# quokka-astro/quokka

Measured on AMD Instinct MI355X. Metric: Mcell-updates/s on 3D Sedov unigrid, higher is better.
Workload: dtype f64; 1 GPU; 3D Sedov blast 256x256x256 unigrid (tests/blast_unigrid_256.in scaled to 256^3 cells per GPU), 128^3 boxes, PPM+HLLC RK2, gamma=1.4, CFL 0.3, reflecting octant; cells_per_gpu=16777216, boxes_per_gpu=8, parallelism=box-decomposition x1, rk2_mode=carry, fofc_stages=0, retries=0, x_sweep_in_y_march=True

## Files before the change

quokka_amd/csrc/qk_hydro_fused.hip:

```cpp
#include "qk_device.hpp"
#include <algorithm>
#include <cmath>
#include <cstdlib>
#include <type_traits>
#include <vector>

#include "qk_internal.hpp"

using namespace qk;

namespace
{

constexpr int NG = 4;

template <class P> QK_DEV void streamStore(P *p, double v) { __builtin_nontemporal_store(v, p); }
template <class P> QK_DEV auto streamLoad(P *p) -> double { return __builtin_nontemporal_load(p); }

struct SGeom {
	int64_t off;
	int glo[3];
	int n[3];
	int pitch;
	int64_t ncell;
};

enum { S_AUX = 0, S_RHS = 4 };
constexpr auto scratchComps(int nscalars) -> int { return S_RHS + NVAR + nscalars + 1; }
constexpr int QK_FUSED_MAX_SCALARS = 3;

struct SweepArgs {
	const qk_box *boxes;
	const SGeom *geom;
	double *scratch;
	int64_t total_cells;
	const qk_array4 *U_in;
	const qk_array4 *U_old;
	qk_array4 *U_out;
	qk_array4 *halfFlux;
	qk_array4 *halfVel;
	qk_iarray4 *redoFlag;
	unsigned long long *redo_count;
	int *error_flag;
	double *max_signal;
	double inv_dx;
	double dx;
	double inv_dx0, dx0;
	double dx3[3];
	double dt;
	double densityFloor, tempFloor;
	double K_visc;
	int use_dual_energy;
	bool reconstruct_eint;
	bool same_old;
	bool store_rk2;
	qk_array4 *rk2Flux;
	qk_array4 *rhs1;
	const qk_carray4 *fluxMask;
	int nseg;
	bool prim_in, prim_out;
	bool store_vel;
	qk_array4 *rk2Vel;
};

QK_DEV auto sarr(SweepArgs const &a, int comp) -> double * { return a.scratch + static_cast<int64_t>(comp) * a.total_cells; }

#ifndef QK_PT_Y
#define QK_PT_Y 7
#define QK_PT_THREADS 512
#endif
constexpr int PT_X = 66, PT_Y = QK_PT_Y, PT_THREADS = QK_PT_THREADS;
constexpr int PT_OWN = PT_X * PT_Y;
constexpr int PT_HALO_Y = 6 * PT_X;
constexpr int PT_HALO = PT_HALO_Y + 6 * PT_Y;
static_assert(PT_HALO <= PT_THREADS && PT_OWN <= PT_THREADS, "one halo cell per thread");

struct PlaneCell {
	double rho, vx, vy, vz, P;
};

struct PlaneRaw {
	double rho, mx, my, mz, E;
};
QK_DEV auto planeLoad(RA4 const &U, int64_t u) -> PlaneRaw
{
	PlaneRaw r;
	r.rho = U.p[u + U.ns * RHO];
	r.mx = U.p[u + U.ns * MX];
	r.my = U.p[u + U.ns * MY];
	r.mz = U.p[u + U.ns * MZ];
	r.E = U.p[u + U.ns * ENE];
	return r;
}
QK_DEV auto planeCell(Eos const &eos, bool re, PlaneRaw const &r) -> PlaneCell
{
	PlaneCell c;
	c.rho = r.rho;
	const Recip R = recipOf(c.rho);
	c.vx = divBy(r.mx, R);
	c.vy = divBy(r.my, R);
	c.vz = divBy(r.mz, R);
	if (eos.isothermal) {
		c.P = c.rho * (eos.cs_iso * eos.cs_iso);
		return c;
	}
	const double kinetic_energy = 0.5 * c.rho * (c.vx * c.vx + c.vy * c.vy + c.vz * c.vz);
	const double Eint_cons = r.E - kinetic_energy;
	if (re) {
		const double e = divBy(Eint_cons, R);
		const double e2 = (c.rho == 0.0) ? 0.0 : divBy(c.rho * e, R);
		c.P = eos.gm1 * c.rho * e2;
	} else {
		const double e = (c.rho == 0.0) ? 0.0 : divBy(Eint_cons, R);
		c.P = eos.gm1 * c.rho * e;
	}
	return c;
}

QK_DEV auto chiCompressive(double Pm2, double Pm1, double Pp1, double Pp2, Recip const &RKS, Recip const &Rbeta) -> double
{
	constexpr double beta_max = 0.85;
	constexpr double Zmax = 0.75;
	constexpr double Zmin = 0.25;
	const double dP1 = fabs(Pp1 - Pm1);
	const double beta_denom = fabs(Pp2 - Pm2);
	const double beta = (beta_denom != 0) ? divBy(dP1, recipOf(beta_denom)) : 0;
	const double chi_min = smax0(smin1(divBy(beta_max - beta, Rbeta)));
	const double Z = divBy(dP1, RKS);
	return smax(chi_min, smin1((Zmax - Z) / (Zmax - Zmin)));
}

template <bool PRIM>
__global__ void __launch_bounds__(PT_THREADS, 4) k_pre3(const qk_box *boxes, const SGeom *geom, const qk_array4 *U_t, double *scratch, int64_t T, Eos eos, bool re, int nseg,
							    int xt, int yt, int ndim)
{
	constexpr bool prim_in = PRIM;
	const unsigned nblk = gridDim.x, lin = blockIdx.x;
	const unsigned q8 = nblk / 8, r8 = nblk % 8, xcd = lin % 8, slot = lin / 8;
	const unsigned logical = (xcd < r8) ? xcd * (q8 + 1) + slot : r8 * (q8 + 1) + (xcd - r8) * q8 + slot;
	const int bix = static_cast<int>(logical % xt), biy = static_cast<int>((logical / xt) % yt), biz = static_cast<int>(logical / (xt * yt));
	__shared__ double s_P[PT_Y + 6][PT_X + 6];
	__shared__ double s_vx[PT_Y][PT_X + 4], s_vy[PT_Y + 4][PT_X];
	__shared__ double s_cx[PT_Y][PT_X + 2], s_cy[PT_Y + 2][PT_X];

	const int b = biz / nseg;
	const int seg = biz - b * nseg;
	const qk_box bx = boxes[b];
	const SGeom g = geom[b];
	RA4 U(U_t[b]);
	const int t = threadIdx.x;
	const int x0 = bx.lo[0] - 1 + bix * PT_X;
	const int y0 = bx.lo[1] - 1 + biy * PT_Y;
	if (x0 > bx.hi[0] + 1 || y0 > bx.hi[1] + 1) {
		return;
	}
	const int nall = bx.hi[2] - bx.lo[2] + 3;
	const int seglen = (nall + nseg - 1) / nseg;
	const int zfirst = bx.lo[2] - 1 + seg * seglen;
	const int zlast = min(zfirst + seglen - 1, bx.hi[2] + 1);
	if (zlast < zfirst) {
		return;
	}
	const int ngy = (ndim >= 2) ? NG : 0, ngz = (ndim == 3) ? NG : 0;
	const int flo[2] = {bx.lo[0] - NG, bx.lo[1] - ngy}, fhi[2] = {bx.hi[0] + NG, bx.hi[1] + ngy};
	const int fzlo = bx.lo[2] - ngz, fzhi = bx.hi[2] + ngz;

	const bool own = t < PT_OWN;
	const int ty = own ? t / PT_X : 0;
	const int tx = own ? t - ty * PT_X : 0;
	const int oi = x0 + tx, oj = y0 + ty;
	const bool ownIn = own && oi <= fhi[0] && oj >= flo[1] && oj <= fhi[1];
	const bool ownOut = own && oi <= bx.hi[0] + 1 && oj <= bx.hi[1] + 1;
	const int h = t - (PT_THREADS - PT_HALO);
	int hx = 0, hy = 0;
	if (h >= 0) {
		if (h < PT_HALO_Y) {
			const int r = h / PT_X;
			hx = h - r * PT_X;
			hy = (r < 3) ? r - 3 : PT_Y + r - 3;
		} else {
			const int r = (h - PT_HALO_Y) / 6, c = (h - PT_HALO_Y) - r * 6;
			hy = r;
			hx = (c < 3) ? c - 3 : PT_X + c - 3;
		}
	}
	const int hi_ = x0 + hx, hj = y0 + hy;
	const bool haloIn = (h >= 0) && hi_ >= flo[0] && hi_ <= fhi[0] && hj >= flo[1] && hj <= fhi[1];
	const bool rimX = (h >= 0) && (hx == -1 || hx == PT_X);
	const bool rimY = (h >= 0) && (hy == -1 || hy == PT_Y);
	const int rx = hx, ry = hy;

	double Pz[5] = {1., 1., 1., 1., 1.}, vzw[5] = {0., 0., 0., 0., 0.}, rhoz[3] = {1., 1., 1.}, chz[3] = {1., 1., 1.};
	const Recip Rbeta = recipOf(0.85 - 0.75);
	double fm[4] = {1., 1., 1., 1.}, fdx[4] = {0., 0., 0., 0.}, fdy[4] = {0., 0., 0., 0.};
	double *Sout = scratch + g.off;
	const PlaneRaw neutral{1., 0., 0., 0., prim_in ? 1. : 1. / eos.gm1};
	auto cellOf = [&](PlaneRaw const &r) -> PlaneCell { return prim_in ? PlaneCell{r.rho, r.mx, r.my, r.mz, r.E} : planeCell(eos, re, r); };
	int64_t uo = ownIn ? U.idx(oi, oj, zfirst - 3) : 0;
	int64_t uh = haloIn ? U.idx(hi_, hj, zfirst - 3) : 0;

	for (int k = zfirst - 3; k <= zlast + 3; ++k, uo += U.ks, uh += U.ks) {
		const bool inPlane = (k >= zfirst) && (k <= zlast);
		const bool kIn = (k >= fzlo) && (k <= fzhi);
		const PlaneCell c = cellOf((ownIn && kIn) ? planeLoad(U, uo) : neutral);
#pragma unroll
		for (int m = 0; m < 4; ++m) {
			Pz[m] = Pz[m + 1];
			vzw[m] = vzw[m + 1];
		}
		Pz[4] = c.P;
		vzw[4] = c.vz;
		rhoz[0] = rhoz[1];
		rhoz[1] = rhoz[2];
		rhoz[2] = c.rho;
#pragma unroll
		for (int m = 0; m < 3; ++m) {
			fm[m] = fm[m + 1];
			fdx[m] = fdx[m + 1];
			fdy[m] = fdy[m + 1];
		}
		if (inPlane) {
			PlaneCell hc{1., 0., 0., 0., 1.};
			if (own) {
				s_P[ty + 3][tx + 3] = c.P;
				s_vx[ty][tx + 2] = c.vx;
				s_vy[ty + 2][tx] = c.vy;
			}
			if (h >= 0) {
				if constexpr (PRIM) {
					if (haloIn && kIn) {
						hc.P = U.p[uh + U.ns * ENE];
						if (hy >= 0 && hy < PT_Y && hx >= -2 && hx < PT_X + 2) {
							hc.vx = U.p[uh + U.ns * MX];
						}
						if (hx >= 0 && hx < PT_X && hy >= -2 && hy < PT_Y + 2) {
							hc.vy = U.p[uh + U.ns * MY];
						}
						if (rimX || rimY) {
							hc.rho = U.p[uh + U.ns * RHO];
						}
					}
				} else {
					hc = cellOf((haloIn && kIn) ? planeLoad(U, uh) : neutral);
				}
				s_P[hy + 3][hx + 3] = hc.P;
				if (hy >= 0 && hy < PT_Y && hx >= -2 && hx < PT_X + 2) {
					s_vx[hy][hx + 2] = hc.vx;
				}
				if (hx >= 0 && hx < PT_X && hy >= -2 && hy < PT_Y + 2) {
					s_vy[hy + 2][hx] = hc.vy;
				}
			}
			__syncthreads();
			if (own) {
				const bool cx = s_vx[ty][tx + 3] < s_vx[ty][tx + 1];
				const bool cy = (ndim >= 2) && (s_vy[ty + 3][tx] < s_vy[ty + 1][tx]);
				double chx = 1.0, chy = 1.0;
				if (cx || cy) {
					const Recip RKS = recipOf(flatteningKS(eos, c.rho, c.P));
					if (cx) {
						const double *Pr = &s_P[ty + 3][tx + 3];
						chx = chiCompressive(Pr[-2], Pr[-1], Pr[1], Pr[2], RKS, Rbeta);
					}
					if (cy) {
						chy = chiCompressive(s_P[ty + 1][tx + 3], s_P[ty + 2][tx + 3], s_P[ty + 4][tx + 3], s_P[ty + 5][tx + 3], RKS, Rbeta);
					}
				}
				s_cx[ty][tx + 1] = chx;
				s_cy[ty + 1][tx] = chy;
			}
			if (rimX) {
				double chx = 1.0;
				if (s_vx[ry][rx + 3] < s_vx[ry][rx + 1]) {
					const double *Pr = &s_P[ry + 3][rx + 3];
					chx = chiCompressive(Pr[-2], Pr[-1], Pr[1], Pr[2], recipOf(flatteningKS(eos, hc.rho, hc.P)), Rbeta);
				}
				s_cx[ry][rx + 1] = chx;
			} else if (rimY) {
				double chy = 1.0;
				if ((ndim >= 2) && (s_vy[ry + 3][rx] < s_vy[ry + 1][rx])) {
					chy = chiCompressive(s_P[ry + 1][rx + 3], s_P[ry + 2][rx + 3], s_P[ry + 4][rx + 3], s_P[ry + 5][rx + 3],
							     recipOf(flatteningKS(eos, hc.rho, hc.P)), Rbeta);
				}
				s_cy[ry + 1][rx] = chy;
			}
			__syncthreads();
			if (own) {
				const double mx = smin(smin(s_cx[ty][tx], s_cx[ty][tx + 1]), s_cx[ty][tx + 2]);
				const double my = smin(smin(s_cy[ty][tx], s_cy[ty + 1][tx]), s_cy[ty + 2][tx]);
				fm[3] = smin(mx, my);
				fdx[3] = smin(s_vx[ty][tx + 3] - c.vx, c.vx - s_vx[ty][tx + 1]);
				fdy[3] = smin(s_vy[ty + 3][tx] - c.vy, c.vy - s_vy[ty + 1][tx]);
			}
			__syncthreads();
		}
		chz[0] = chz[1];
		chz[1] = chz[2];
		chz[2] = 1.0;
		if ((ndim == 3) && (vzw[3] < vzw[1])) {
			chz[2] = chiCompressive(Pz[0], Pz[1], Pz[3], Pz[4], recipOf(flatteningKS(eos, rhoz[0], Pz[2])), Rbeta);
		}
		const int ko = k - 3;
		if (ko >= zfirst && ko <= zlast && ownOut) {
			const int64_t cc = (oi - g.glo[0]) + static_cast<int64_t>(g.pitch) * ((oj - g.glo[1]) + static_cast<int64_t>(g.n[1]) * (ko - g.glo[2]));
			Sout[(S_AUX + 0) * T + cc] = smin(fm[0], smin(smin(chz[0], chz[1]), chz[2]));
			Sout[(S_AUX + 1) * T + cc] = fdx[0];
			Sout[(S_AUX + 2) * T + cc] = fdy[0];
			Sout[(S_AUX + 3) * T + cc] = smin(vzw[2] - vzw[1], vzw[1] - vzw[0]);
		}
	}
}

template <int ORDER> QK_DEV void cellEdges(const double qm2, const double qm1, const double q0, const double qp1, const double qp2, double &am, double &ap)
{
	if (ORDER == 3) {
		ppmEdges(qm2, qm1, q0, qp1, qp2, am, ap);
	} else if (ORDER == 2) {
		plmEdges<QK_LIMITER_MINMOD>(qm1, q0, qp1, am, ap);
	} else {
		am = q0;
		ap = q0;
	}
}

QK_DEV void flattenEdges(double chi, double mean, double &am, double &ap)
{
	am = chi * am + (1. - chi) * mean;
	ap = chi * ap + (1. - chi) * mean;
}

template <int ORDER> QK_DEV void reconstructVar(double chi, double qm2, double qm1, double q0, double qp1, double qp2, double &am, double &ap)
{
	cellEdges<ORDER>(qm2, qm1, q0, qp1, qp2, am, ap);
	flattenEdges(chi, q0, am, ap);
}
template <int ORDER, int NV, class NB> QK_DEV void reconstructCell(double chi, const double (&q0)[NV], NB nb, double (&am)[NV], double (&ap)[NV])
{
#pragma unroll
	for (int n = 0; n < NV; ++n) {
		reconstructVar<ORDER>(chi, nb(-2, n), nb(-1, n), q0[n], nb(1, n), nb(2, n), am[n], ap[n]);
	}
}

template <int NV, int W> QK_DEV void getColumn(const double (*s)[W], int t, double (&v)[NV])
{
#pragma unroll
	for (int n = 0; n < NV; ++n) {
		v[n] = s[n][t];
	}
}
template <int NV, int W> QK_DEV void putColumn(double (*s)[W], int t, const double (&v)[NV])
{
#pragma unroll
	for (int n = 0; n < NV; ++n) {
		s[n][t] = v[n];
	}
}

template <int NS> QK_DEV void primsOf(RA4 const &U, int64_t u, Eos const &eos, bool re, bool prim_in, const double (&Uc)[NVAR], double (&q)[NVAR + NS])
{
	if (prim_in) {
#pragma unroll
		for (int n = 0; n < NVAR; ++n) {
			q[n] = Uc[n];
		}
	} else {
		consToPrim(eos, re, Uc, q);
	}
#pragma unroll
	for (int n = NVAR; n < NVAR + NS; ++n) {
		q[n] = U.p[u + U.ns * n];
	}
}
template <int NS> QK_DEV void loadPrims(RA4 const &U, int64_t u, Eos const &eos, bool re, bool prim_in, double (&q)[NVAR + NS], double (&Uc)[NVAR])
{
#pragma unroll
	for (int n = 0; n < NVAR; ++n) {
		Uc[n] = U.p[u + U.ns * n];
	}
	primsOf<NS>(U, u, eos, re, prim_in, Uc, q);
}

template <int DIR, int RIEMANN, bool TWOD, int NS>
QK_DEV void faceFluxAll(Eos const &eos, bool re, int ndim, const double (&qL)[NVAR + NS], const double (&qR)[NVAR + NS], double du, double dvl, double dvr, double dwl,
			double dwr, double K_visc, double (&F)[NVAR + NS], double &vf)
{
	Wave wv;
	faceFlux<DIR, RIEMANN, TWOD>(eos, re, ndim, qL, qR, du, dvl, dvr, dwl, dwr, K_visc, F, vf, NS > 0 ? &wv : nullptr);
#pragma unroll
	for (int n = NVAR; n < NVAR + NS; ++n) {
		F[n] = scalarFlux<RIEMANN>(wv, qL[n], qR[n]);
	}
}

using CA4 = A4<const char, qk_carray4>;
QK_DEV auto maskByte(qk_carray4 const &d, int i, int j, int k) -> int
{
	if (i < d.begin[0] || i >= d.end[0] || j < d.begin[1] || j >= d.end[1] || k < d.begin[2] || k >= d.end[2]) {
		return 0;
	}
	return CA4(d)(i, j, k);
}
template <int STAGE, int NV> QK_DEV void maskedFaceFlux(SweepArgs const &a, int b, int i, int j, int k, const double F[NV])
{
	if (STAGE == 1) {
		WA4 HF(a.halfFlux[b]);
		const int64_t o = HF.idx(i, j, k);
#pragma unroll
		for (int n = 0; n < NV; ++n) {
			HF.p[o + HF.ns * n] = F[n];
		}
	} else {
		RA4 HF(a.halfFlux[b]);
		WA4 RF(a.rk2Flux[b]);
		const int64_t o = HF.idx(i, j, k), o2 = RF.idx(i, j, k);
#pragma unroll
		for (int n = 0; n < NV; ++n) {
			RF.p[o2 + RF.ns * n] = 0.5 * HF.p[o + HF.ns * n] + 0.5 * F[n];
		}
	}
}

template <int NV> QK_DEV void loadF1(SweepArgs const &a, int b, const int (&fi)[3], double (&F1)[NV + 1])
{
	RA4 HF(a.halfFlux[b]);
	RA4 HV(a.halfVel[b]);
	const int64_t o = HF.idx(fi[0], fi[1], fi[2]);
#pragma unroll
	for (int n = 0; n < NV; ++n) {
		F1[n] = HF.p[o + HF.ns * n];
	}
	F1[NV] = HV(fi[0], fi[1], fi[2]);
}
template <int STAGE, bool CARRY, bool FOFC, int DIR, int NS, bool TWOD>
QK_DEV void settleFace(SweepArgs const &a, Eos const &eos, int ndim, int b, const int (&fi)[3], bool live, bool marked, const double (&F1)[NVAR + NS + 1],
		       const double (&qLo)[NVAR + NS], const double (&qRo)[NVAR + NS], double (&F)[NVAR + NS], double &vf)
{
	constexpr int NV = NVAR + NS;
	if (CARRY) {
		if (marked) {
			maskedFaceFlux<STAGE, NV>(a, b, fi[0], fi[1], fi[2], F);
		}
		return;
	}
	int fm[3] = {fi[0], fi[1], fi[2]};
	fm[DIR] -= 1;
	bool firstOrder = false;
	if constexpr (FOFC) {
		CIA4 flag(a.redoFlag[b]);
		firstOrder = (flag(fm[0], fm[1], fm[2]) != 0) || (flag(fi[0], fi[1], fi[2]) != 0);
	}
	if (STAGE == 2) {
#pragma unroll
		for (int n = 0; n < NV; ++n) {
			F[n] = 0.5 * F1[n] + 0.5 * F[n];
		}
		vf = 0.5 * F1[NV] + 0.5 * vf;
	}
	if constexpr (FOFC) {
		if (firstOrder) {
			if (STAGE == 1) {
				faceFluxAll<DIR, QK_RIEMANN_LLF, TWOD, NS>(eos, a.reconstruct_eint, ndim, qLo, qRo, 0., 0., 0., 0., 0., 0., F, vf);
			} else {
				RA4 Uold(a.U_old[b]);
				double qL[NV], qR[NV], Uc[NVAR];
				loadPrims<NS>(Uold, Uold.idx(fm[0], fm[1], fm[2]), eos, a.reconstruct_eint, false, qL, Uc);
				loadPrims<NS>(Uold, Uold.idx(fi[0], fi[1], fi[2]), eos, a.reconstruct_eint, false, qR, Uc);
				faceFluxAll<DIR, QK_RIEMANN_LLF, TWOD, NS>(eos, a.reconstruct_eint, ndim, qL, qR, 0., 0., 0., 0., 0., 0., F, vf);
			}
		}
	} else if (STAGE == 1) {
		if (live) {
			WA4 HF(a.halfFlux[b]);
			WA4 HV(a.halfVel[b]);
			const int64_t o = HF.idx(fi[0], fi[1], fi[2]);
#pragma unroll
			for (int n = 0; n < NV; ++n) {
				HF.p[o + HF.ns * n] = F[n];
			}
			HV(fi[0], fi[1], fi[2]) = vf;
		}
	}
	if (STAGE == 2 && a.store_rk2 && live) {
		WA4 RF(a.rk2Flux[b]);
		const int64_t o2 = RF.idx(fi[0], fi[1], fi[2]);
#pragma unroll
		for (int n = 0; n < NV; ++n) {
			RF.p[o2 + RF.ns * n] = F[n];
		}
	}
	if (STAGE == 2 && a.store_vel && live) {
		WA4 RV(a.rk2Vel[b]);
		RV(fi[0], fi[1], fi[2]) = vf;
	}
}

QK_DEV void reduceSignal(double *max_signal, double sig0, double sig1)
{
	for (int off = 32; off > 0; off >>= 1) {
		sig0 = smax(sig0, __shfl_xor(sig0, off));
		sig1 = smax(sig1, __shfl_xor(sig1, off));
	}
	if ((threadIdx.x & 63) == 0) {
		atomicMaxNonNeg(&max_signal[0], sig0);
		atomicMaxNonNeg(&max_signal[1], sig1);
	}
}
template <int NDIM> QK_DEV auto cellCentredDivV(RA4 const &U, int i, int j, int k, const double dx[3]) -> double
{
	auto vel = [&](int ii, int jj, int kk, int d) { return U(ii, jj, kk, MX + d) / U(ii, jj, kk, RHO); };
	double s = (vel(i + 1, j, k, 0) - vel(i - 1, j, k, 0)) / dx[0];
	if (NDIM >= 2) {
		s = s + (vel(i, j + 1, k, 1) - vel(i, j - 1, k, 1)) / dx[1];
	}
	if (NDIM == 3) {
		s = s + (vel(i, j, k + 1, 2) - vel(i, j, k - 1, 2)) / dx[2];
	}
	return 0.5 * s;
}

struct EpiConst {
	Recip RkB, RkBu, Rmu;
};
QK_DEV auto epiConst(Eos const &eos) -> EpiConst
{
	EpiConst c;
	c.RkB = eos.RkB;
	c.RkBu = eos.RkBu;
	c.Rmu = eos.Rmu;
	return c;
}
QK_DEV auto epiTgas(Eos const &eos, EpiConst const &ec, Recip const &Rrho, double Eint) -> double
{
	if (eos.tmodel == 1) {
		return sqrt(sqrt(4.0 * Eint / eos.alpha));
	}
	const double e = divBy(Eint, Rrho);
	const double T = divBy(e * eos.mu * Eos::m_u * eos.gm1, ec.RkB);
	return divBy(T * Eos::k_B, ec.RkBu);
}
QK_DEV auto epiEint(Eos const &eos, EpiConst const &ec, double rho, double T) -> double
{
	if (eos.tmodel == 1) {
		return (eos.alpha / 4.0) * ((T * T) * (T * T));
	}
	const double p = divBy(rho * T * Eos::k_B, ec.Rmu);
	const double e = p / (eos.gm1 * rho);
	return divBy(e * rho * eos.kB_user, ec.RkB);
}

template <int NS, int CS, bool FOFC = false, int NDIM = 3>
QK_DEV void updateCellFrom(SweepArgs const &a, Eos const &eos, EpiConst const &ec, int b, int i, int j, int k, double U[NVAR + NS], const double rhs_sweeps[NVAR + NS],
			   double div_v, const double half[NVAR + NS + 1], double &sig0, double &sig1, bool haveP = false, double Pknown = 0.)
{
	WA4 Un(a.U_out[b]);
	IA4 flag(a.redoFlag[b]);
	if constexpr (FOFC) {
		if (flag(i, j, k) != 0) {
			div_v = cellCentredDivV<NDIM>(RA4(a.U_old[b]), i, j, k, a.dx3);
		}
	}
	double rhs[NVAR + NS];
#pragma unroll
	for (int n = 0; n < NVAR + NS; ++n) {
		rhs[n] = rhs_sweeps[n];
	}
	double Pgas;
	if (CS == 2) {
		Pgas = half[NVAR + NS];
	} else if (haveP) {
		Pgas = Pknown;
	} else {
		const double rho = U[RHO];
		if (eos.isothermal) {
			Pgas = rho * eos.cs_iso * eos.cs_iso;
		} else {
			const Recip Ro = recipOf(rho);
			const double vx = divBy(U[MX], Ro), vy = divBy(U[MY], Ro), vz = divBy(U[MZ], Ro);
			const double thermal_energy = U[ENE] - 0.5 * rho * (vx * vx + vy * vy + vz * vz);
			const double e = (rho == 0.0) ? 0.0 : divBy(thermal_energy, Ro);
			Pgas = eos.gm1 * rho * e;
		}
	}
	double r[NVAR];
#pragma unroll
	for (int n = 0; n < NVAR; ++n) {
		r[n] = rhs[n];
	}
	r[EINT] += -Pgas * div_v;
	if (CS == 1) {
		WA4 R1(a.rhs1[b]);
		const int64_t c1 = R1.idx(i, j, k);
		const double hdt = 0.5 * a.dt;
#pragma unroll
		for (int n = 0; n < NVAR + NS; ++n) {
			streamStore(&R1.p[c1 + R1.ns * n], U[n] + hdt * ((n < NVAR) ? r[n] : rhs[n]));
		}
		streamStore(&R1.p[c1 + R1.ns * (NVAR + NS)], Pgas);
	}
	if (CS == 2) {
		const double hdt = 0.5 * a.dt;
#pragma unroll
		for (int n = 0; n < NVAR + NS; ++n) {
			U[n] = half[n] + hdt * ((n < NVAR) ? r[n] : rhs[n]);
		}
	} else {
#pragma unroll
		for (int n = 0; n < NVAR; ++n) {
			U[n] = U[n] + a.dt * r[n];
		}
#pragma unroll
		for (int n = NVAR; n < NVAR + NS; ++n) {
// ... 319 lines not shown
	pos[0] = i;
	pos[OT] = ot;
	pos[DIR] = lo - 3;
	int64_t c = (pos[0] - g.glo[0]) * st[0] + (pos[1] - g.glo[1]) * st[1] + (pos[2] - g.glo[2]) * st[2];
	const double *S = a.scratch + g.off;
	double *Sw = a.scratch + g.off;
	RA4 Uin(a.U_in[b]);
	RA4 Uold(a.U_old[b]);
	const EpiConst ec = epiConst(eos);
	int64_t u = Uin.idx(pos[0], pos[1], pos[2]);
	const int64_t ums = (DIR == 1) ? Uin.js : Uin.ks;

	constexpr int AV = Axes<DIR, TWOD>::v, AW = Axes<DIR, TWOD>::w;
	double q[5][NV];
	double apPrev[NV], Fprev[NV];
	double vfPrev = 0., dVprev = 0., dWprev = 0.;
	bool maskCol = false;
	int maskLo = 0, maskHi = -1;
	if (CARRY && a.fluxMask != nullptr) {
		const qk_carray4 md = a.fluxMask[b];
		maskCol = live && i >= md.begin[0] && i < md.end[0] && ot >= md.begin[OT] && ot < md.end[OT];
		maskLo = md.begin[DIR];
		maskHi = md.end[DIR] - 1;
	}
	constexpr bool RING = LAST && (STAGE == 1);
	__shared__ double s_ring[RING ? 3 : 1][RING ? NV : 1][RING ? 64 * MARCH_BY : 1];
	__shared__ double s_fx[FUSEX ? MARCH_BY : 1][FUSEX ? NV + 2 : 1][FUSEX ? XW : 1];
	__shared__ double s_edge[FUSEX ? MARCH_BY : 1][FUSEX ? XROWS : 1][6][FUSEX ? NV + 1 : 1];
	double chiPrev = 1.;
	const int lself = (FUSEX && threadIdx.x == 0) ? 69 : static_cast<int>(threadIdx.x) + 2;
	const int lnext = (FUSEX && threadIdx.x == 63) ? 68 : static_cast<int>(threadIdx.x) + 3;
	const int tid = threadIdx.y * 64 + threadIdx.x;
	const bool ring = RING && a.same_old;
	int slot = 0;
	double Uo[NV];
#pragma unroll
	for (int n = 0; n < NV; ++n) {
		apPrev[n] = 0.;
		Fprev[n] = 0.;
#pragma unroll
		for (int m = 0; m < 5; ++m) {
			q[m][n] = 0.;
		}
	}

	constexpr bool PFQ = !FUSEX && NS == 0;
	double Un[NVAR];
	if constexpr (PFQ) {
#pragma unroll
		for (int n = 0; n < NVAR; ++n) {
			Un[n] = Uin.p[u + Uin.ns * n];
		}
	}
	for (int step = 0; step < nvalid + 6; ++step, c += ms, u += ums) {
#pragma unroll
		for (int n = 0; n < NV; ++n) {
			q[0][n] = q[1][n];
			q[1][n] = q[2][n];
			q[2][n] = q[3][n];
			q[3][n] = q[4][n];
		}
		{
			double Uc[NVAR];
			if constexpr (PFQ) {
#pragma unroll
				for (int n = 0; n < NVAR; ++n) {
					Uc[n] = Un[n];
					Un[n] = Uin.p[u + ums + Uin.ns * n];
				}
				primsOf<NS>(Uin, u, eos, a.reconstruct_eint, a.prim_in, Uc, q[4]);
			} else {
				loadPrims<NS>(Uin, u, eos, a.reconstruct_eint, a.prim_in, q[4], Uc);
			}
			if constexpr (RING) {
				if (ring) {
#pragma unroll
					for (int n = 0; n < NV; ++n) {
						Uo[n] = s_ring[slot][n][tid];
						s_ring[slot][n][tid] = (n < NVAR) ? Uc[n] : q[4][n];
					}
					slot = (slot == 2) ? 0 : slot + 1;
				}
			}
		}
		if (step < 4) {
			continue;
		}
		const int64_t cc = c - 2 * ms;
		const double chi = S[(S_AUX + 0) * T + cc];
		const double dV = S[(S_AUX + 1 + AV) * T + cc];
		const double dW = S[(S_AUX + 1 + AW) * T + cc];
		int fidx[3], cidx[3];
		fidx[0] = cidx[0] = i;
		fidx[OT] = cidx[OT] = ot;
		fidx[DIR] = lo + (step - 5);
		cidx[DIR] = lo + (step - 6);
		const int64_t cu = cc - ms;
		double rhs_in[NV + 1], F1[NV + 1];
		if (step >= 6) {
			if constexpr (FUSEX) {
				double(*sx)[XW] = s_fx[threadIdx.y];
				EdgeRow<NV> *edge = s_edge[threadIdx.y];
				const int rr = (step - 6) & (XROWS - 1);
				if (rr == 0) {
					fusexEdgeBatch<ORDER, NS>(a, eos, Uin, g, st, S, bx.lo[0] + bix * 64, cidx[DIR], hi, ot, edge);
					waveFence();
					stageEdgeRow<NV>(sx, edge[0]);
				}
				const double Dy = S[(S_AUX + 2) * T + cu];
				const int l = static_cast<int>(threadIdx.x) + 2;
				putColumn(sx, l, q[1]);
				waveFence();
				double amx[NV], apx[NV];
				reconstructCell<ORDER>(chiPrev, q[1], [&](int m, int n) { return sx[n][l + m]; }, amx, apx);
				const double uLeft = sx[PVX][l - 1];
				waveFence();
				putColumn(sx, l, apx);
				sx[NV][l] = Dy;
				sx[NV + 1][l] = dVprev;
				waveFence();
				double qLx[NV], Fx[NV], vfx;
				getColumn(sx, l - 1, qLx);
				const double dvl = sx[NV][l - 1], dwl = sx[NV + 1][l - 1];
				faceFluxAll<0, QK_RIEMANN_HLLC, false, NS>(eos, a.reconstruct_eint, 3, qLx, amx, q[1][PVX] - uLeft, dvl, Dy, dwl, dVprev, a.K_visc, Fx, vfx);
				waveFence();
				putColumn(sx, l, Fx);
				sx[NV][l] = vfx;
				waveFence();
#pragma unroll
				for (int n = 0; n < NV; ++n) {
					rhs_in[n] = a.inv_dx0 * (sx[n][lself] - sx[n][lnext]);
				}
				rhs_in[NV] = (sx[NV][lnext] - sx[NV][lself]) / a.dx0;
				waveFence();
				if (rr + 1 < XROWS) {
					stageEdgeRow<NV>(sx, edge[rr + 1]);
				}
			} else {
#pragma unroll
				for (int n = 0; n < NV + 1; ++n) {
					rhs_in[n] = streamLoad(&S[(S_RHS + n) * T + cu]);
				}
			}
			if (LAST && !ring && !(CARRY && STAGE == 2)) {
				const int64_t co = Uold.idx(cidx[0], cidx[1], cidx[2]);
#pragma unroll
				for (int n = 0; n < NV; ++n) {
					Uo[n] = Uold.p[co + Uold.ns * n];
				}
			}
			if (CARRY && LAST && STAGE == 2) {
				RA4 R1(a.rhs1[b]);
				const int64_t c1 = R1.idx(cidx[0], cidx[1], cidx[2]);
#pragma unroll
				for (int n = 0; n < NV + 1; ++n) {
					F1[n] = R1.p[c1 + R1.ns * n];
				}
			}
		}
		if (!CARRY && STAGE == 2 && step >= 5) {
			loadF1<NV>(a, b, fidx, F1);
		}
		double am[NV], ap[NV];
		reconstructCell<ORDER>(chi, q[2], [&](int m, int n) { return q[2 + m][n]; }, am, ap);
		if (step >= 5) {
			const double du = q[2][PVX + DIR] - q[1][PVX + DIR];
			double F[NV], vf;
			faceFluxAll<DIR, QK_RIEMANN_HLLC, TWOD, NS>(eos, a.reconstruct_eint, TWOD ? 2 : 3, apPrev, am, du, dVprev, dV, dWprev, dW, a.K_visc, F, vf);
			bool marked = false;
			if (maskCol && fidx[DIR] >= maskLo && cidx[DIR] <= maskHi) {
				CA4 M(a.fluxMask[b]);
				const int m0 = (cidx[DIR] >= maskLo) ? M(cidx[0], cidx[1], cidx[2]) : 0;
				const int m1 = (fidx[DIR] <= maskHi) ? M(fidx[0], fidx[1], fidx[2]) : 0;
				marked = (m0 | m1) != 0;
			}
			settleFace<STAGE, CARRY, FOFC, DIR, NS, TWOD>(a, eos, TWOD ? 2 : 3, b, fidx, live, marked, F1, q[1], q[2], F, vf);
			if (step >= 6) {
				double rhs[NV];
#pragma unroll
				for (int n = 0; n < NV; ++n) {
					rhs[n] = rhs_in[n] + a.inv_dx * (Fprev[n] - F[n]);
				}
				const double div_v = rhs_in[NV] + (vf - vfPrev) / a.dx;
				if (LAST) {
					if (live) {
						updateCellFrom<NS, CARRY ? STAGE : 0, FOFC, TWOD ? 2 : 3>(a, eos, ec, b, cidx[0], cidx[1], cidx[2], Uo, rhs, div_v, F1, sig0, sig1,
													    (STAGE == 1) && a.same_old && !a.reconstruct_eint && !a.prim_in, q[1][PPRES]);
					}
				} else if (live) {
#pragma unroll
					for (int n = 0; n < NV; ++n) {
						streamStore(&Sw[(S_RHS + n) * T + cu], rhs[n]);
					}
					streamStore(&Sw[RHS_DIVV * T + cu], div_v);
				}
			}
#pragma unroll
			for (int n = 0; n < NV; ++n) {
				Fprev[n] = F[n];
			}
			vfPrev = vf;
		}
#pragma unroll
		for (int n = 0; n < NV; ++n) {
			apPrev[n] = ap[n];
		}
		dVprev = dV;
		dWprev = dW;
		chiPrev = chi;
	}
	if (LAST && a.max_signal != nullptr) {
		reduceSignal(a.max_signal, sig0, sig1);
	}
}

inline auto smallLevelCells() -> int64_t
{
	static const int64_t v = [] {
		const char *e = std::getenv("QK_SMALL_LEVEL_CELLS");
		return (e != nullptr) ? static_cast<int64_t>(std::atoll(e)) : static_cast<int64_t>(2) << 20;
	}();
	return v;
}

inline auto smallMinLen() -> int
{
	static const int v = [] {
		const char *e = std::getenv("QK_SMALL_MINLEN");
		return (e != nullptr) ? std::max(1, std::atoi(e)) : 4;
	}();
	return v;
}

auto marchSegments(const qk_level *lev, int dir, int ot) -> int
{
	if (const char *e = std::getenv("QK_MARCH_SEGMENTS")) {
		return std::max(1, std::atoi(e));
	}
	const int64_t cols = static_cast<int64_t>(lev->nboxes) * lev->maxlen[0] * lev->maxlen[ot];
	const int64_t want = (131072 + cols - 1) / std::max<int64_t>(cols, 1);
	const int minlen = (cols * lev->maxlen[dir] < smallLevelCells()) ? smallMinLen() : 16;
	const int cap = std::max(1, lev->maxlen[dir] / minlen);
	return static_cast<int>(std::min<int64_t>(std::max<int64_t>(want, 1), std::min(cap, 16)));
}

inline auto rowAlign() -> bool
{
	static const bool v = [] {
		const char *e = std::getenv("QK_ROW_ALIGN");
		return e == nullptr || std::atoi(e) == 1 || std::atoi(e) == 3;
	}();
	return v;
}

auto scratchGeom(const qk_level *lev, std::vector<SGeom> &g) -> int64_t
{
	g.resize(lev->nboxes);
	const bool al = rowAlign();
	int64_t off = 0;
	for (int b = 0; b < lev->nboxes; ++b) {
		for (int d = 0; d < 3; ++d) {
			g[b].glo[d] = lev->boxes[b].lo[d] - NG;
			g[b].n[d] = lev->boxes[b].hi[d] - lev->boxes[b].lo[d] + 1 + 2 * NG;
		}
		g[b].pitch = al ? (g[b].n[0] + 15) / 16 * 16 : g[b].n[0];
		if (al) {
			off = (off + 15) / 16 * 16 + (16 - NG);
		}
		g[b].off = off;
		g[b].ncell = static_cast<int64_t>(g[b].pitch) * g[b].n[1] * g[b].n[2];
		off += g[b].ncell;
	}
	return al ? (off + 15) / 16 * 16 : off;
}

auto buildGeom(qk_level *lev) -> int
{
	if (lev->d_sgeom != nullptr) {
		return QK_OK;
	}
	std::vector<SGeom> g;
	const int64_t total = scratchGeom(lev, g);
	void *d = nullptr;
	QK_HIP_CHECK(lev->ctx, hipMalloc(&d, sizeof(SGeom) * lev->nboxes));
	QK_HIP_CHECK(lev->ctx, hipMemcpy(d, g.data(), sizeof(SGeom) * lev->nboxes, hipMemcpyHostToDevice));
	lev->d_sgeom = d;
	lev->sgeom_total_cells = total;
	return QK_OK;
}

auto prePassSegments(const qk_level *lev, int xt, int yt) -> int
{
	if (const char *e = std::getenv("QK_PRE_SEGMENTS")) {
		return std::max(1, std::atoi(e));
	}
	const bool small = static_cast<int64_t>(lev->nboxes) * lev->maxlen[0] * lev->maxlen[1] * lev->maxlen[2] < smallLevelCells();
	const int64_t tiles = static_cast<int64_t>(xt) * yt * lev->nboxes;
	const int nplanes = lev->maxlen[2] + 2;
	if (small) {
		return static_cast<int>(std::min<int64_t>((1024 + tiles - 1) / tiles, std::max(1, nplanes / smallMinLen())));
	}
	const int base = std::max(1, std::min(8, (nplanes + 15) / 30));
	int nseg = base;
	const double slots = 512.0;
	if (static_cast<double>(tiles) * base / slots < 6.0) {
		double best = 1e300;
		for (int c = std::max(1, base - 1); c <= base + 1; ++c) {
			const double rounds = static_cast<double>(tiles) * c / slots;
			const int seglen = (nplanes + c - 1) / c;
			const double cost = (std::ceil(rounds) / rounds) * (static_cast<double>(seglen + 6) / seglen);
			if (cost < best) {
				best = cost;
				nseg = c;
			}
		}
	}
	return nseg;
}

auto sweepArgsFor(SweepArgs a, const qk_hydro_stage_args *args, int d) -> SweepArgs
{
	a.halfFlux = args->halfFlux[d];
	a.halfVel = args->halfVel[d];
	a.rk2Flux = args->fluxRk2[d];
	a.rk2Vel = args->velRk2[d];
	a.inv_dx = 1.0 / args->dx[d];
	a.dx = args->dx[d];
	return a;
}

auto fusexApplies(const qk_level *lev, SweepArgs const &a, bool carry, int nscalars) -> bool
{
	const char *e = std::getenv("QK_FUSEX");
	if (!carry || nscalars != 0 || lev->ndim != 3 || a.fluxMask != nullptr || (e != nullptr && std::atoi(e) == 0)) {
		return false;
	}
	for (int b = 0; b < lev->nboxes; ++b) {
		if ((lev->boxes[b].hi[0] - lev->boxes[b].lo[0] + 1) % 64 != 0) {
			return false;
		}
	}
	return true;
}

template <int ORDER, int STAGE, int NS, bool CARRY, bool FOFC = false> void launchSweeps(qk_level *lev, hipStream_t s, SweepArgs a, Eos eos, const qk_hydro_stage_args *args)
{
	const bool fusex = fusexApplies(lev, a, CARRY, NS);
	if (!fusex) {
		const SweepArgs ax = sweepArgsFor(a, args, 0);
		const int64_t slab = static_cast<int64_t>(lev->maxlen[0] + 2 * NG) * lev->maxlen[1];
		const dim3 grid(static_cast<unsigned>((slab + XOUT - 1) / XOUT), static_cast<unsigned>(lev->maxlen[2]), static_cast<unsigned>(lev->nboxes));
		ProfScope ps(lev->ctx, s, "k_sweep_x");
		if (lev->ndim == 3) {
			hipLaunchKernelGGL((k_sweep_x<ORDER, STAGE, NS, CARRY, 3, FOFC>), grid, dim3(XB), 0, s, ax, eos);
		} else if constexpr (!CARRY) {
			if (lev->ndim == 2) {
				hipLaunchKernelGGL((k_sweep_x<ORDER, STAGE, NS, false, 2, FOFC>), grid, dim3(XB), 0, s, ax, eos);
			} else {
				hipLaunchKernelGGL((k_sweep_x<ORDER, STAGE, NS, false, 1, FOFC>), grid, dim3(XB), 0, s, ax, eos);
			}
		}
	}
	if (lev->ndim == 1) {
		return;
	}
	{
		SweepArgs ay = sweepArgsFor(a, args, 1);
		ay.same_old = (lev->ndim == 2) && (args->U_in == args->U_old);
		ay.nseg = marchSegments(lev, 1, 2);
		ay.inv_dx0 = 1.0 / args->dx[0];
		ay.dx0 = args->dx[0];
		const dim3 grid((lev->maxlen[0] + 63) / 64, (lev->maxlen[2] + MARCH_BY - 1) / MARCH_BY, lev->nboxes * ay.nseg);
		ProfScope ps(lev->ctx, s, fusex ? "k_sweep_xy" : "k_sweep_y");
		if (lev->ndim == 2) {
			if constexpr (!CARRY) {
				hipLaunchKernelGGL((k_sweep_march<1, ORDER, STAGE, true, NS, false, true, FOFC>), grid, dim3(64, MARCH_BY), 0, s, ay, eos);
			}
			return;
		}
		if constexpr (CARRY && !FOFC && NS == 0) {
			if (fusex) {
				hipLaunchKernelGGL((k_sweep_march<1, ORDER, STAGE, false, NS, CARRY, false, FOFC, true>), grid, dim3(64, MARCH_BY), 0, s, ay, eos);
			}
		}
		if (!fusex) {
			hipLaunchKernelGGL((k_sweep_march<1, ORDER, STAGE, false, NS, CARRY, false, FOFC>), grid, dim3(64, MARCH_BY), 0, s, ay, eos);
		}
	}
	{
		SweepArgs az = sweepArgsFor(a, args, 2);
		az.same_old = (args->U_in == args->U_old);
		az.nseg = marchSegments(lev, 2, 1);
		const dim3 grid((lev->maxlen[0] + 63) / 64, (lev->maxlen[1] + MARCH_BY - 1) / MARCH_BY, lev->nboxes * az.nseg);
		ProfScope ps(lev->ctx, s, "k_sweep_z");
		hipLaunchKernelGGL((k_sweep_march<2, ORDER, STAGE, true, NS, CARRY, false, FOFC>), grid, dim3(64, MARCH_BY), 0, s, az, eos);
	}
}

template <int ORDER, int NS> void launchStage(qk_level *lev, hipStream_t s, SweepArgs const &a, Eos const &eos, const qk_hydro_stage_args *args)
{
	auto form = [&](auto stage) {
		constexpr int STAGE = decltype(stage)::value;
		if (args->fofc_pass != 0) {
			launchSweeps<ORDER, STAGE, NS, false, true>(lev, s, a, eos, args);
		} else if (args->rk2_carry_rhs != 0) {
			launchSweeps<ORDER, STAGE, NS, true>(lev, s, a, eos, args);
		} else {
			launchSweeps<ORDER, STAGE, NS, false>(lev, s, a, eos, args);
		}
	};
	if (args->stage == 1) {
		form(std::integral_constant<int, 1>{});
	} else {
		form(std::integral_constant<int, 2>{});
	}
}
template <int ORDER> void launchOrder(int nscalars, qk_level *lev, hipStream_t s, SweepArgs const &a, Eos const &eos, const qk_hydro_stage_args *args)
{
	switch (nscalars) {
	case 0: return launchStage<ORDER, 0>(lev, s, a, eos, args);
	case 1: return launchStage<ORDER, 1>(lev, s, a, eos, args);
	case 2: return launchStage<ORDER, 2>(lev, s, a, eos, args);
	default: return launchStage<ORDER, 3>(lev, s, a, eos, args);
	}
}

}

extern "C" {

int64_t qk_hydro_stage_scratch_bytes(qk_level *lev, const qk_hydro_traits *t)
{
	if (lev == nullptr) {
		return QK_ERR_INVALID;
	}
	if (int rc = checkTraits(lev->ctx, t); rc != QK_OK) {
		return rc;
	}
	std::vector<SGeom> g;
	const int64_t cells = scratchGeom(lev, g);
	return cells * scratchComps(t->nscalars) * static_cast<int64_t>(sizeof(double));
}

int qk_hydro_stage_fused(qk_level *lev, qk_stream stream, const qk_hydro_traits *t, const qk_hydro_stage_args *args)
{
	if (lev == nullptr) {
		return QK_ERR_INVALID;
	}
	qk_ctx *ctx = lev->ctx;
	if (int rc = checkTraits(ctx, t); rc != QK_OK) {
		return rc;
	}
	if (int rc = needsLibraryEos(ctx, t, "qk_hydro_stage_fused (EnforceLimits)"); rc != QK_OK) {
		return rc;
	}
	QK_REQUIRE(ctx, args != nullptr, "qk_hydro_stage_fused: NULL args");
	if (lev->nboxes == 0) {
		return QK_OK;
	}
	if (t->nscalars > QK_FUSED_MAX_SCALARS || t->nmscalars != 0) {
		return setError(ctx, QK_ERR_UNSUPPORTED, "qk_hydro_stage_fused: up to 3 passive scalars, no mass scalars (use the reference-shaped operators)");
	}
	if (t->ndim != lev->ndim) {
		return setError(ctx, QK_ERR_INVALID, "qk_hydro_stage_fused: traits.ndim differs from the level's dimension");
	}
	if (t->ndim != 3 && args->rk2_carry_rhs != 0) {
		return setError(ctx, QK_ERR_UNSUPPORTED, "qk_hydro_stage_fused: rk2_carry_rhs is instantiated for 3-D builds");
	}
	QK_REQUIRE(ctx, args->K_visc >= 0.0, "qk_hydro_stage_fused: negative artificial-viscosity coefficient");
	QK_REQUIRE(ctx, args->stage == 1 || args->stage == 2, "qk_hydro_stage_fused: stage must be 1 or 2");
	QK_REQUIRE(ctx, args->reconstruction_order >= 1 && args->reconstruction_order <= 3, "qk_hydro_stage_fused: reconstruction_order must be 1..3");
	QK_REQUIRE(ctx, args->U_in && args->U_old && args->U_out && args->redoFlag && args->d_redo_count && args->d_error_flag && args->scratch,
		   "qk_hydro_stage_fused: NULL array");
	QK_REQUIRE(ctx, args->fofc_pass == 0 || (args->K_visc == 0.0 && (args->rk2_carry_rhs == 0 || args->stage == 1)),
		   "qk_hydro_stage_fused: the fused first-order flux correction pass needs K_visc == 0 and, in the carried-rhs form, stage 1 (use the reference-shaped operators otherwise)");
	QK_REQUIRE(ctx, args->rk2_carry_rhs == 0 || (args->rhs1 != nullptr && args->store_flux_rk2 == 0),
		   "qk_hydro_stage_fused: rk2_carry_rhs needs rhs1 and excludes store_flux_rk2 (flux_rk2 is formed on the faces flux_mask marks, nowhere else)");
	if (args->rk2_carry_rhs != 0 && args->flux_mask != nullptr) {
		for (int d = 0; d < t->ndim; ++d) {
			QK_REQUIRE(ctx, args->halfFlux[d] != nullptr && args->fluxRk2[d] != nullptr && args->fluxRk2[d] != args->halfFlux[d],
				   "qk_hydro_stage_fused: flux_mask needs halfFlux[d] and a distinct fluxRk2[d]");
		}
	}
	for (int d = 0; d < t->ndim; ++d) {
		QK_REQUIRE(ctx, args->rk2_carry_rhs != 0 || (args->halfFlux[d] && args->halfVel[d]), "qk_hydro_stage_fused: NULL halfFlux/halfVel");
		QK_REQUIRE(ctx, args->store_flux_rk2 == 0 || args->stage != 2 || (args->fluxRk2[d] != nullptr && args->fluxRk2[d] != args->halfFlux[d]),
			   "qk_hydro_stage_fused: store_flux_rk2 needs fluxRk2[d], distinct from halfFlux[d]");
		QK_REQUIRE(ctx, lev->maxlen[d] >= 1, "qk_hydro_stage_fused: empty box");
	}
	if (args->store_vel_rk2 != 0) {
		QK_REQUIRE(ctx, args->rk2_carry_rhs == 0, "qk_hydro_stage_fused: store_vel_rk2 excludes rk2_carry_rhs (the carried form has no halfVel to average with)");
		QK_REQUIRE(ctx, args->stage == 2, "qk_hydro_stage_fused: store_vel_rk2 belongs to stage 2 (stage 1 leaves its face velocity in halfVel)");
		for (int d = 0; d < t->ndim; ++d) {
			QK_REQUIRE(ctx, args->velRk2[d] != nullptr, "qk_hydro_stage_fused: store_vel_rk2 needs velRk2[d]");
			QK_REQUIRE(ctx, args->velRk2[d] != args->halfVel[d],
				   "qk_hydro_stage_fused: store_vel_rk2 needs velRk2[d] distinct from halfVel[d] (the x sweep evaluates a tile-boundary face in both tiles, and both need v1 intact)");
		}
	}
	QK_REQUIRE(ctx, args->scratch_bytes >= qk_hydro_stage_scratch_bytes(lev, t), "qk_hydro_stage_fused: scratch too small");
	if (args->prim_in != 0 || args->prim_out != 0) {
		QK_REQUIRE(ctx, t->reconstruct_eint == 0 && !Eos(*t).isothermal && t->eos_temperature_model == 0,
			   "qk_hydro_stage_fused: the primitive hand-off is the gamma-law, reconstruct_eint = 0 form");
		QK_REQUIRE(ctx, args->fofc_pass == 0, "qk_hydro_stage_fused: the primitive hand-off has no correction pass (redo the step without it)");
		QK_REQUIRE(ctx, (args->prim_out == 0 || args->stage == 1) && (args->prim_in == 0 || (args->stage == 2 && args->U_in != args->U_old)),
			   "qk_hydro_stage_fused: prim_out belongs to stage 1, prim_in to stage 2 (whose old state is a different array)");
	}

	if (int rc = buildGeom(lev); rc != QK_OK) {
		return rc;
	}
	auto s = static_cast<hipStream_t>(stream);
	const Eos eos(*t);
	const bool re = (t->reconstruct_eint != 0);
	auto *scratch = static_cast<double *>(args->scratch);
	const int64_t T = lev->sgeom_total_cells;
	const SGeom *geom = static_cast<const SGeom *>(lev->d_sgeom);
	const qk_box *boxes = lev->d_boxes;

	{
		ProfScope ps(ctx, s, "k_pre");
		const int xt = (lev->maxlen[0] + 2 + PT_X - 1) / PT_X, yt = (lev->maxlen[1] + 2 + PT_Y - 1) / PT_Y;
		const int nseg = prePassSegments(lev, xt, yt);
		const dim3 grid(static_cast<unsigned>(xt) * yt * lev->nboxes * nseg);
		if (args->prim_in != 0) {
			hipLaunchKernelGGL(k_pre3<true>, grid, dim3(PT_THREADS), 0, s, boxes, geom, args->U_in, scratch, T, eos, re, nseg, xt, yt, t->ndim);
		} else {
			hipLaunchKernelGGL(k_pre3<false>, grid, dim3(PT_THREADS), 0, s, boxes, geom, args->U_in, scratch, T, eos, re, nseg, xt, yt, t->ndim);
		}
	}

	SweepArgs a{};
	a.boxes = boxes;
	a.geom = geom;
	a.scratch = scratch;
	a.total_cells = T;
	a.U_in = args->U_in;
	a.U_old = args->U_old;
	a.U_out = args->U_out;
	a.redoFlag = args->redoFlag;
	a.redo_count = reinterpret_cast<unsigned long long *>(args->d_redo_count);
	a.error_flag = args->d_error_flag;
	a.max_signal = args->d_max_signal;
	a.dt = args->dt;
	a.densityFloor = args->densityFloor;
	a.tempFloor = args->tempFloor;
	a.K_visc = args->K_visc;
	a.use_dual_energy = args->use_dual_energy;
	a.reconstruct_eint = re;
	a.store_rk2 = (args->store_flux_rk2 != 0);
	a.store_vel = (args->store_vel_rk2 != 0);
	a.rhs1 = args->rhs1;
	a.fluxMask = (args->rk2_carry_rhs != 0) ? args->flux_mask : nullptr;
	a.prim_in = (args->prim_in != 0);
	a.prim_out = (args->prim_out != 0);
	for (int d = 0; d < 3; ++d) {
		a.dx3[d] = args->dx[d];
	}

	if (args->reconstruction_order == 3) {
		launchOrder<3>(t->nscalars, lev, s, a, eos, args);
	} else if (args->reconstruction_order == 2) {
		launchOrder<2>(t->nscalars, lev, s, a, eos, args);
	} else {
		launchOrder<1>(t->nscalars, lev, s, a, eos, args);
	}
	QK_HIP_CHECK(ctx, hipGetLastError());
	return QK_OK;
}

}
```

Baseline: 3333 Mcell-updates/s.

## Prefetch next z-plane loads and enlarge flattening pre-pass tiles

The flattening pre-pass now issues the global loads for plane k+1 right after the first barrier of plane k, so the loads overlap the shared-memory chi computation. The per-thread fm/fdx/fdy shift registers move into a 3-deep shared-memory ring to free registers. The tile height and block size are doubled (15 rows, 1024 threads) and the segment heuristic's slot count is halved to match the larger blocks. The risks are occupancy loss from more shared memory and registers per block, and fewer blocks available to cover the GPU.

```diff
diff --git a/quokka_amd/csrc/qk_hydro_fused.hip b/quokka_amd/csrc/qk_hydro_fused.hip
--- a/quokka_amd/csrc/qk_hydro_fused.hip
+++ b/quokka_amd/csrc/qk_hydro_fused.hip
@@ -66,8 +66,8 @@
 QK_DEV auto sarr(SweepArgs const &a, int comp) -> double * { return a.scratch + static_cast<int64_t>(comp) * a.total_cells; }
 
 #ifndef QK_PT_Y
-#define QK_PT_Y 7
-#define QK_PT_THREADS 512
+#define QK_PT_Y 15
+#define QK_PT_THREADS 1024
 #endif
 constexpr int PT_X = 66, PT_Y = QK_PT_Y, PT_THREADS = QK_PT_THREADS;
 constexpr int PT_OWN = PT_X * PT_Y;
@@ -192,17 +192,51 @@
 
 	double Pz[5] = {1., 1., 1., 1., 1.}, vzw[5] = {0., 0., 0., 0., 0.}, rhoz[3] = {1., 1., 1.}, chz[3] = {1., 1., 1.};
 	const Recip Rbeta = recipOf(0.85 - 0.75);
-	double fm[4] = {1., 1., 1., 1.}, fdx[4] = {0., 0., 0., 0.}, fdy[4] = {0., 0., 0., 0.};
+	__shared__ double s_fm[3][PT_OWN], s_fdx[3][PT_OWN], s_fdy[3][PT_OWN];
+	int ring = 0;
 	double *Sout = scratch + g.off;
 	const PlaneRaw neutral{1., 0., 0., 0., prim_in ? 1. : 1. / eos.gm1};
 	auto cellOf = [&](PlaneRaw const &r) -> PlaneCell { return prim_in ? PlaneCell{r.rho, r.mx, r.my, r.mz, r.E} : planeCell(eos, re, r); };
+	const bool hasVx = hy >= 0 && hy < PT_Y && hx >= -2 && hx < PT_X + 2;
+	const bool hasVy = hx >= 0 && hx < PT_X && hy >= -2 && hy < PT_Y + 2;
+	PlaneRaw ro = neutral, rh = neutral;
+	auto request = [&](int kn, int64_t uon, int64_t uhn) {
+		ro = neutral;
+		rh = neutral;
+		if (kn > zlast + 3 || kn < fzlo || kn > fzhi) {
+			return;
+		}
+		if (ownIn) {
+			ro = planeLoad(U, uon);
+		}
+		if (haloIn && kn >= zfirst && kn <= zlast) {
+			if constexpr (PRIM) {
+				rh.E = U.p[uhn + U.ns * ENE];
+				if (hasVx) {
+					rh.mx = U.p[uhn + U.ns * MX];
+				}
+				if (hasVy) {
+					rh.my = U.p[uhn + U.ns * MY];
+				}
+				if (rimX || rimY) {
+					rh.rho = U.p[uhn + U.ns * RHO];
+				}
+			} else {
+				rh = planeLoad(U, uhn);
+			}
+		}
+	};
 	int64_t uo = ownIn ? U.idx(oi, oj, zfirst - 3) : 0;
 	int64_t uh = haloIn ? U.idx(hi_, hj, zfirst - 3) : 0;
-
-	for (int k = zfirst - 3; k <= zlast + 3; ++k, uo += U.ks, uh += U.ks) {
+	request(zfirst - 3, uo, uh);
+
+	for (int k = zfirst - 3; k <= zlast + 3; ++k) {
 		const bool inPlane = (k >= zfirst) && (k <= zlast);
-		const bool kIn = (k >= fzlo) && (k <= fzhi);
-		const PlaneCell c = cellOf((ownIn && kIn) ? planeLoad(U, uo) : neutral);
+		const PlaneCell c = cellOf(ro);
+		PlaneCell hc{1., 0., 0., 0., 1.};
+		if (inPlane && h >= 0) {
+			hc = cellOf(rh);
+		}
 #pragma unroll
 		for (int m = 0; m < 4; ++m) {
 			Pz[m] = Pz[m + 1];
@@ -213,45 +247,39 @@
 		rhoz[0] = rhoz[1];
 		rhoz[1] = rhoz[2];
 		rhoz[2] = c.rho;
-#pragma unroll
-		for (int m = 0; m < 3; ++m) {
-			fm[m] = fm[m + 1];
-			fdx[m] = fdx[m + 1];
-			fdy[m] = fdy[m + 1];
-		}
+		chz[0] = chz[1];
+		chz[1] = chz[2];
+		chz[2] = 1.0;
+		if ((ndim == 3) && (vzw[3] < vzw[1])) {
+			chz[2] = chiCompressive(Pz[0], Pz[1], Pz[3], Pz[4], recipOf(flatteningKS(eos, rhoz[0], Pz[2])), Rbeta);
+		}
+		const int ko = k - 3;
+		if (ko >= zfirst && ko <= zlast && ownOut) {
+			const int64_t cc = (oi - g.glo[0]) + static_cast<int64_t>(g.pitch) * ((oj - g.glo[1]) + static_cast<int64_t>(g.n[1]) * (ko - g.glo[2]));
+			Sout[(S_AUX + 0) * T + cc] = smin(s_fm[ring][t], smin(smin(chz[0], chz[1]), chz[2]));
+			Sout[(S_AUX + 1) * T + cc] = s_fdx[ring][t];
+			Sout[(S_AUX + 2) * T + cc] = s_fdy[ring][t];
+			Sout[(S_AUX + 3) * T + cc] = smin(vzw[2] - vzw[1], vzw[1] - vzw[0]);
+		}
+		uo += U.ks;
+		uh += U.ks;
 		if (inPlane) {
-			PlaneCell hc{1., 0., 0., 0., 1.};
 			if (own) {
 				s_P[ty + 3][tx + 3] = c.P;
 				s_vx[ty][tx + 2] = c.vx;
 				s_vy[ty + 2][tx] = c.vy;
 			}
 			if (h >= 0) {
-				if constexpr (PRIM) {
-					if (haloIn && kIn) {
-						hc.P = U.p[uh + U.ns * ENE];
-						if (hy >= 0 && hy < PT_Y && hx >= -2 && hx < PT_X + 2) {
-							hc.vx = U.p[uh + U.ns * MX];
-						}
-						if (hx >= 0 && hx < PT_X && hy >= -2 && hy < PT_Y + 2) {
-							hc.vy = U.p[uh + U.ns * MY];
-						}
-						if (rimX || rimY) {
-							hc.rho = U.p[uh + U.ns * RHO];
-						}
-					}
-				} else {
-					hc = cellOf((haloIn && kIn) ? planeLoad(U, uh) : neutral);
-				}
 				s_P[hy + 3][hx + 3] = hc.P;
-				if (hy >= 0 && hy < PT_Y && hx >= -2 && hx < PT_X + 2) {
+				if (hasVx) {
 					s_vx[hy][hx + 2] = hc.vx;
 				}
-				if (hx >= 0 && hx < PT_X && hy >= -2 && hy < PT_Y + 2) {
+				if (hasVy) {
 					s_vy[hy + 2][hx] = hc.vy;
 				}
 			}
 			__syncthreads();
+			request(k + 1, uo, uh);
 			if (own) {
 				const bool cx = s_vx[ty][tx + 3] < s_vx[ty][tx + 1];
 				const bool cy = (ndim >= 2) && (s_vy[ty + 3][tx] < s_vy[ty + 1][tx]);
@@ -288,26 +316,16 @@
 			if (own) {
 				const double mx = smin(smin(s_cx[ty][tx], s_cx[ty][tx + 1]), s_cx[ty][tx + 2]);
 				const double my = smin(smin(s_cy[ty][tx], s_cy[ty + 1][tx]), s_cy[ty + 2][tx]);
-				fm[3] = smin(mx, my);
-				fdx[3] = smin(s_vx[ty][tx + 3] - c.vx, c.vx - s_vx[ty][tx + 1]);
-				fdy[3] = smin(s_vy[ty + 3][tx] - c.vy, c.vy - s_vy[ty + 1][tx]);
+				s_fm[ring][t] = smin(mx, my);
+				s_fdx[ring][t] = smin(s_vx[ty][tx + 3] - c.vx, c.vx - s_vx[ty][tx + 1]);
+				s_fdy[ring][t] = smin(s_vy[ty + 3][tx] - c.vy, c.vy - s_vy[ty + 1][tx]);
 			}
 			__syncthreads();
 		}
-		chz[0] = chz[1];
-		chz[1] = chz[2];
-		chz[2] = 1.0;
-		if ((ndim == 3) && (vzw[3] < vzw[1])) {
-			chz[2] = chiCompressive(Pz[0], Pz[1], Pz[3], Pz[4], recipOf(flatteningKS(eos, rhoz[0], Pz[2])), Rbeta);
-		}
-		const int ko = k - 3;
-		if (ko >= zfirst && ko <= zlast && ownOut) {
-			const int64_t cc = (oi - g.glo[0]) + static_cast<int64_t>(g.pitch) * ((oj - g.glo[1]) + static_cast<int64_t>(g.n[1]) * (ko - g.glo[2]));
-			Sout[(S_AUX + 0) * T + cc] = smin(fm[0], smin(smin(chz[0], chz[1]), chz[2]));
-			Sout[(S_AUX + 1) * T + cc] = fdx[0];
-			Sout[(S_AUX + 2) * T + cc] = fdy[0];
-			Sout[(S_AUX + 3) * T + cc] = smin(vzw[2] - vzw[1], vzw[1] - vzw[0]);
-		}
+		else {
+			request(k + 1, uo, uh);
+		}
+		ring = (ring == 2) ? 0 : ring + 1;
 	}
 }
 
@@ -1233,7 +1251,7 @@
 	}
 	const int base = std::max(1, std::min(8, (nplanes + 15) / 30));
 	int nseg = base;
-	const double slots = 512.0;
+	const double slots = 256.0;
 	if (static_cast<double>(tiles) * base / slots < 6.0) {
 		double best = 1e300;
 		for (int c = std::max(1, base - 1); c <= base + 1; ++c) {
```

Result: no change. 3315 Mcell-updates/s (-0.5%).
